# Intelligent-Driving-Laboratory/GOPS

Measured on AMD Instinct MI355X. Metric: env-model steps/sec (batch x H), FHADP compute_gradient + update, higher is better.
Workload: dtype f32; 1 GPU; target_veh3dof_fhadp_b4096_h30; env_id=pyth_veh3dofconti, algorithm=FHADP, batch_per_gpu=4096, horizon=30, activation=elu, parallelism=dp1

## Files before the change

### gops_amd/csrc/api.hip

```cpp
#include <math.h>
#include <stdio.h>
#include <stdlib.h>
#include <string.h>

#include <algorithm>
#include <mutex>
#include <vector>

#include "common.h"
#include "launchers.h"
#include "rollout_choice.h"

bool lds_attr_needed(const void* kernel) {
    static std::mutex mu;
    static std::vector<const void*> seen;
    std::lock_guard<std::mutex> lk(mu);
    for (const void* k : seen)
        if (k == kernel) return false;
    seen.push_back(kernel);
    return true;
}

namespace {

// ... 61 lines not shown
    return buf != nullptr ? buf + 16 * slot : nullptr;
#else
    (void)slot;
    return nullptr;
#endif
}

int check_mlp(const GopsMlp& m, int in_dim, int out_dim, bool f16) {
    if (m.n_layers < 2 || m.n_layers > GOPS_MAX_LAYERS) return GOPS_ERR_UNSUPPORTED;
    if (m.sizes[0] != in_dim || m.sizes[m.n_layers] != out_dim) return GOPS_ERR_BAD_ARG;
    if (out_dim < 1 || out_dim > GOPS_MAX_ACT) return GOPS_ERR_UNSUPPORTED;
    for (int j = 1; j < m.n_layers; ++j)
        if (m.sizes[j] < 16 || (m.sizes[j] & (f16 ? 63 : 15))) return GOPS_ERR_UNSUPPORTED;
    if (m.hidden_act < GOPS_ACT_LINEAR || m.hidden_act > GOPS_ACT_TANH) return GOPS_ERR_BAD_ARG;
    for (int j = 0; j < m.n_layers; ++j)
        if (m.weight[j] == nullptr || m.bias[j] == nullptr) return GOPS_ERR_BAD_ARG;
    return GOPS_OK;
}

void fill_mlp(MlpDev& d, const GopsMlp& m) {
    memset(&d, 0, sizeof(d));
    d.nl = m.n_layers;
    d.act = m.hidden_act;
    for (int j = 0; j <= m.n_layers; ++j) d.dims[j] = m.sizes[j];
    for (int j = 0; j < m.n_layers; ++j) {
        d.kp[j] = pad16(m.sizes[j]);
        d.kp32[j] = pad32(m.sizes[j]);
        d.w[j] = m.weight[j];
        d.b[j] = m.bias[j];
    }
}

void carve_packs(Carver& c, MlpDev& d, bool f16) {
    for (int j = 0; j < d.nl - 1; ++j) {
        if (f16) {
            const size_t n = ((size_t)d.dims[j + 1] * d.kp32[j] + 1) / 2;
            d.wph[j] = reinterpret_cast<const f16x8*>(c.take(n));
            d.wpth[j] = reinterpret_cast<const f16x8*>(c.take(n));
            continue;
        }
        const size_t n = (size_t)d.dims[j + 1] * d.kp[j];
        d.wp[j] = reinterpret_cast<const f32x4*>(c.take(n));
        d.wpt[j] = reinterpret_cast<const f32x4*>(c.take(n));
    }
}

struct Plan {
    RolloutParams p;
    RolloutChoice choice;
    RolloutParams* dev_params = nullptr;
    DwLayer dw[GOPS_MAX_LAYERS];
    float* dw_part[GOPS_MAX_LAYERS] = {};
    float* dw_part_b[GOPS_MAX_LAYERS] = {};
    float* dummy = nullptr;
    size_t dummy_floats = 0;
    size_t bytes = 0;
};

int build_plan(const GopsRolloutDesc& desc, void* ws, Plan& plan) {
    RolloutParams& p = plan.p;
    memset(&p, 0, sizeof(p));
    const GopsEnv& e = desc.env;
    if (desc.batch < 1 || desc.horizon < 1 || desc.horizon > GOPS_MAX_HORIZON) return GOPS_ERR_BAD_ARG;
    if (desc.variant_flags & ~GOPS_VF_ALL) return GOPS_ERR_BAD_ARG;
    if (e.kind < GOPS_ENV_NONE || e.kind > GOPS_ENV_MOBILEROBOT) return GOPS_ERR_BAD_ARG;
    if (e.obs_dim < 1 || e.data_env) return GOPS_ERR_BAD_ARG;
    const int pol_out = (e.kind == GOPS_ENV_NONE) ? 1 : e.act_dim;
    if (desc.dtype != GOPS_DTYPE_F32 && desc.dtype != GOPS_DTYPE_F16) return GOPS_ERR_BAD_ARG;
    const bool f16 = desc.dtype == GOPS_DTYPE_F16;
    int rc = GOPS_OK;
    if (desc.open_loop) {
        if (e.kind == GOPS_ENV_NONE || desc.tail_value || desc.finite_horizon || f16) return GOPS_ERR_BAD_ARG;
    } else if ((rc = check_mlp(desc.policy, e.obs_dim + (desc.finite_horizon ? 1 : 0), pol_out, f16)) != GOPS_OK) {
        return rc;
    }
    if (desc.tail_value && (rc = check_mlp(desc.value, e.obs_dim, 1, f16)) != GOPS_OK) return rc;
    if (e.kind == GOPS_ENV_NONE && (desc.horizon != 1 || desc.tail_value || desc.finite_horizon)) return GOPS_ERR_BAD_ARG;
    if (e.scale_obs && e.kind != GOPS_ENV_LQ && e.kind != GOPS_ENV_IDPENDULUM && e.kind < GOPS_ENV_CARTPOLE) return GOPS_ERR_UNSUPPORTED;
    if (e.kind == GOPS_ENV_CARTPOLE && (e.obs_dim != 4 || e.act_dim != 1)) return GOPS_ERR_BAD_ARG;
    if (e.kind == GOPS_ENV_PENDULUM && (e.obs_dim != 3 || e.act_dim != 1)) return GOPS_ERR_BAD_ARG;
    if (e.kind == GOPS_ENV_VEH2DOF && (e.act_dim != 1 || e.pre_horizon < 1 || e.obs_dim != 4 + e.pre_horizon || e.clip_obs ||
                                        (e.cstr_err && e.n_constraint != 1))) return GOPS_ERR_BAD_ARG;
    if (e.kind == GOPS_ENV_MOBILEROBOT && (e.obs_dim != MOB_OBS || e.act_dim != 2 || e.n_constraint != 1 || e.scale_obs)) return GOPS_ERR_BAD_ARG;
    if (e.kind >= GOPS_ENV_CARTPOLE && f16) return GOPS_ERR_UNSUPPORTED;
    if (e.kind == GOPS_ENV_LQ && (e.obs_dim > GOPS_MAX_LQ_STATE || e.act_dim > GOPS_MAX_ACT)) return GOPS_ERR_UNSUPPORTED;
    if (e.kind == GOPS_ENV_IDPENDULUM && (e.obs_dim != 6 || e.act_dim != 1 || e.clip_obs)) return GOPS_ERR_BAD_ARG;
    if (e.kind == GOPS_ENV_VEH3DOFCONTI &&
        (e.act_dim != 2 || e.pre_horizon < 1 || e.obs_dim != 6 + 4 * e.pre_horizon || e.clip_obs))
        return GOPS_ERR_BAD_ARG;
    if (e.kind == GOPS_ENV_VEH3DOF_SURR &&
        (e.act_dim != 2 || e.pre_horizon < 1 || e.n_surr < (e.cstr_err ? 0 : 1) || e.n_surr > (e.cstr_err ? 0 : GOPS_MAX_SURR) ||
         (e.cstr_err ? e.n_constraint != 2 : (e.n_constraint != 1 && e.n_constraint != 3)) ||
         e.obs_dim != 6 + 4 * e.pre_horizon + 4 * e.n_surr || e.clip_obs ||
         (e.surr_penalty && (e.n_surr != 1 || e.n_constraint != 1)) ||
         desc.open_loop == 1 || desc.dtype != GOPS_DTYPE_F32))
        return GOPS_ERR_BAD_ARG;
    if (e.clip_obs && e.obs_dim > (e.kind == GOPS_ENV_MOBILEROBOT ? GOPS_MAX_CLIP_OBS : 8)) return GOPS_ERR_UNSUPPORTED;
    if (e.repeat_num < 0 || e.repeat_num > GOPS_MAX_REPEAT) return GOPS_ERR_BAD_ARG;
    if (e.repeat_num > 1 && (f16 || (e.kind != GOPS_ENV_LQ && e.kind != GOPS_ENV_IDPENDULUM && e.kind != GOPS_ENV_CARTPOLE &&
                                     e.kind != GOPS_ENV_PENDULUM)))
        return GOPS_ERR_UNSUPPORTED;

    p.B = desc.batch;
    p.H = desc.horizon;
    p.fh = desc.finite_horizon ? 1 : 0;
    p.need_grad = desc.need_grad ? 1 : 0;
    p.tail = desc.tail_value ? 1 : 0;
    p.tail_unmasked = (desc.tail_value && desc.tail_unmasked) ? 1 : 0;
    p.env = e;
    lq_pad_env(p.env);
    fill_ref_defaults(p.env);
    p.open_loop = desc.open_loop == 2 ? 2 : (desc.open_loop ? 1 : 0);
    p.f16 = f16 ? 1 : 0;
    p.vflags = desc.variant_flags;
    p.dw_wgs = desc.dw_workgroups > 0 ? desc.dw_workgroups : 512;
    if (p.open_loop) {
        GopsMlp dummy;
// ... 238 lines not shown
            const long long nw = (long long)p.pol.dims[j + 1] * p.pol.dims[j], nb = p.pol.dims[j + 1];
            int fw = -1, fb = -1;
            for (int k = 0; k < T.n; ++k) {
                if (T.grad[k] == c.grad->weight[j] && T.numel[k] == nw) fw = k;
                if (T.grad[k] == c.grad->bias[j] && T.numel[k] == nb) fb = k;
            }
            if (fw < 0 || fb < 0 || !T.param[fw] || !T.exp_avg[fw] || !T.exp_avg_sq[fw] || !T.param[fb] || !T.exp_avg[fb] || !T.exp_avg_sq[fb])
                return GOPS_ERR_BAD_ARG;
        }
    }
    if (tail->polyak != nullptr) {
        if (tail->adam == nullptr || tail->polyak->n != tail->adam->n) return GOPS_ERR_BAD_ARG;
        for (int k = 0; k < tail->polyak->n; ++k) {
            bool found = false;
            for (int i = 0; i < tail->adam->n; ++i)
                found = found || (tail->polyak->grad[k] == tail->adam->param[i] && tail->polyak->numel[k] == tail->adam->numel[i]);
            if (!found || tail->polyak->param[k] == nullptr) return GOPS_ERR_BAD_ARG;
        }
    }
    return GOPS_OK;
}

int check_backward_call(const GopsRolloutDesc& desc, const RolloutParams& p, const BackwardCall& c) {
    if ((p.open_loop != 0) != (c.g_head_pre != nullptr)) return GOPS_ERR_BAD_ARG;
    if (p.open_loop && c.in->head_pre == nullptr) return GOPS_ERR_BAD_ARG;
    if (c.ext_delta != nullptr && desc.env.kind != GOPS_ENV_NONE) return GOPS_ERR_BAD_ARG;
    if (!p.open_loop && c.want_params)
        for (int j = 0; j < p.pol.nl - (c.ext_delta != nullptr ? 1 : 0); ++j)
            if (c.grad->weight[j] == nullptr || c.grad->bias[j] == nullptr) return GOPS_ERR_BAD_ARG;
    int rc = GOPS_OK;
    if (c.tail != nullptr && (rc = check_update_tail(desc, p, c)) != GOPS_OK) return rc;
    if (c.adj != nullptr && (p.tail || p.f16)) return GOPS_ERR_UNSUPPORTED;
    const Phase ph(p.vflags);
    if ((ph.only_a || ph.only_b) && (p.open_loop || !c.want_params || c.ext_delta != nullptr || c.adj != nullptr)) return GOPS_ERR_UNSUPPORTED;
    return GOPS_OK;
}

bool choose_dw_stage(Plan& plan, const BackwardCall& c, const SweepCall& call) {
    const RolloutParams& p = plan.p;
    const KernelChoice& sweep = plan.choice.bwd;
    if (p.open_loop || !c.want_params) return true;
    const Phase ph(p.vflags);
    const int L = p.pol.nl - 1;
    const bool own_sweep = c.adj == nullptr && c.ext_delta == nullptr;
    const bool cstr_seeds = !(p.env.kind == GOPS_ENV_VEH3DOF_SURR && p.env.surr_penalty) &&
                            (c.in->grad_constraint != nullptr || c.in->grad_constraint_prod != nullptr || c.in->grad_constraint_step != nullptr);
    const bool scaled = own_sweep && !cstr_seeds;
    for (int j = 0; j < L; ++j) {
        if ((ph.only_a && j == 0) || (ph.only_b && j != 0)) continue;
        if (j == 0 && plan.choice.fuse_dw0 && own_sweep && !(p.vflags & (GOPS_VF_BWD_PHASE_A | GOPS_VF_BWD_PHASE_B))) {
            if (!choose_dw_in_sweep(plan.dw[0], sweep.grid, H64_W0_COLS)) return false;
        } else {
            choose_dw_gemm(plan.dw[j], p.f16 != 0, scaled, p.vflags);
        }
    }
    if (c.ext_delta == nullptr && !ph.only_b) {
        if (!sweep_fuses_out(sweep, call)) choose_dw_out(plan.dw[L], p.f16 != 0);
        else if (!choose_dw_in_sweep(plan.dw[L], sweep.grid, plan.dw[L].K)) return false;
    }
    return true;
}

void fill_patch(Plan& plan, const BackwardCall& c, const SweepCall& call, BwdPatch& q) {
    RolloutParams& p = plan.p;
    const int L = p.pol.nl - 1;
    p.in = *c.in;
    p.grad_v = c.grad_v;
    p.g_head_pre = c.g_head_pre;
    p.ext_delta = c.ext_delta;
    p.ext = call.ext;
    if (c.adj != nullptr) {
        p.adj_gfo = c.adj->grad_final_obs;
        p.adj_gobs = c.adj->grad_obs;
        p.adj_first_only = (c.adj->first_step_only != 0 && p.H > 1) ? 1 : 0;
    }
    p.dbg = dbg_timing_buffer(1);
    if (sweep_fuses_out(plan.choice.bwd, call)) {
        p.sp.out_part = plan.dw_part[L];
        p.sp.out_part_b = plan.dw_part_b[L];
    }
    memset(&q, 0, sizeof(q));
    q.in = *c.in;
    q.grad_v = c.grad_v;
    q.g_head_pre = c.g_head_pre;
    q.ext_delta = c.ext_delta;
    q.adj_gfo = p.adj_gfo;
    q.adj_gobs = p.adj_gobs;
    q.adj_first_only = p.adj_first_only;
    q.out_part = p.sp.out_part;
    q.out_part_b = p.sp.out_part_b;
    q.dbg = p.dbg;
    if (plan.dw[0].kernel == DwKernel::InSweep) {
        q.w0_part = plan.dw_part[0];
        q.w0_part_b = plan.dw_part_b[0];
    }
    if (c.tail != nullptr && c.tail->adam != nullptr) {
        q.ad_st = c.tail->adam_state;
        q.ad_snap = p.gscale + 4;
        q.ad_b1 = c.tail->beta1; q.ad_b2 = c.tail->beta2;
    }
}

hipError_t launch_sweep(const GopsRolloutDesc& desc, const Plan& plan, const BackwardCall& c, const BwdPatch& q, hipStream_t s) {
    const RolloutParams& p = plan.p;
    hipError_t e;
    if (p.adj_first_only && c.want_params) {
        const size_t S0 = (size_t)tiles(p) * TB * p.H;
        for (int j = 1; j < p.pol.nl; ++j)
// ... 7 lines not shown
}

hipError_t launch_dw_layer(const DwLayer& d, const void* D, const void* X, float* part, float* part_b, const float* dscale, int rows,
                           float* gw, float* gb, ReduceJobs& jobs, hipStream_t s) {
    const hipError_t e = launch_dw(d, D, X, part, part_b, dscale, s);
    if (e == hipSuccess) add_reduce_jobs(jobs, d, part, part_b, rows, gw, gb);
    return e;
}

void attach_update_tail(ReduceJobs& jobs, const GopsUpdateTail& tail, const RolloutParams& p) {
    if (tail.adam != nullptr) {
        const GopsAdamTensors& T = *tail.adam;
        for (int i = 0; i < jobs.n; ++i)
            for (int k = 0; k < T.n; ++k)
                if (T.grad[k] == jobs.out[i]) { jobs.ad_p[i] = T.param[k]; jobs.ad_m[i] = T.exp_avg[k]; jobs.ad_v[i] = T.exp_avg_sq[k]; }
        jobs.ad_snap = p.gscale + 4;
        jobs.ad_skipped = &tail.adam_state->skipped_nonfinite;
        jobs.ad_b1 = tail.beta1; jobs.ad_b2 = tail.beta2; jobs.ad_eps = (float)tail.eps;
        if (tail.polyak != nullptr) {
            for (int i = 0; i < jobs.n; ++i)
                for (int k = 0; k < tail.polyak->n; ++k)
                    if (jobs.ad_p[i] != nullptr && tail.polyak->grad[k] == jobs.ad_p[i]) jobs.pk_t[i] = tail.polyak->param[k];
            jobs.pk_omt = (float)(1.0 - tail.polyak_tau);
            jobs.pk_tau = (float)tail.polyak_tau;
        }
    }
    if (tail.mean_x != nullptr) {
        jobs.mean_x = tail.mean_x; jobs.mean_n = tail.mean_n; jobs.mean_sc = (float)tail.mean_scale; jobs.mean_stats = tail.mean_stats;
    }
}

int run_backward(const GopsRolloutDesc& desc, const BackwardCall& c, void* ws, size_t ws_bytes, hipStream_t s) {
    if (!desc.need_grad || c.grad_v == nullptr) return GOPS_ERR_BAD_ARG;
    Plan plan;
    int rc = build_plan(desc, ws, plan);
    if (rc != GOPS_OK) return rc;
    if (ws == nullptr || ws_bytes < plan.bytes) return GOPS_ERR_WORKSPACE;
    const RolloutParams& p = plan.p;
    if ((rc = check_backward_call(desc, p, c)) != GOPS_OK) return rc;
    const SweepCall call{desc.env.repeat_num > 1 || c.adj != nullptr, c.ext_delta != nullptr, c.want_params};
    if (!choose_sweep(p, plan.choice, call, plan.choice.bwd) || !choose_dw_stage(plan, c, call)) return GOPS_ERR_UNSUPPORTED;
    BwdPatch q;
    fill_patch(plan, c, call, q);
    hipError_t e;
    if ((e = launch_sweep(desc, plan, c, q, s)) != hipSuccess) return (int)e;
    dbg_print_backward(p);
    if (p.open_loop || !c.want_params) return (int)launch_fill_zero(p.gscale, 4, s);
    ProfScope scope(desc.env.kind == GOPS_ENV_NONE ? 5 : 2, s);
    ReduceJobs jobs;
    memset(&jobs, 0, sizeof(jobs));
    if (p.f16) jobs.unscale = p.gscale;
    else jobs.poison = reinterpret_cast<const unsigned*>(p.gscale) + 3;
    const int L = p.pol.nl - 1;
    for (int j = 0; j <= L; ++j) {
        const DwLayer& d = plan.dw[j];
        if (d.kernel == DwKernel::None) continue;
        if ((e = launch_dw_layer(d, j < L ? p.st.d[j + 1] : p.st.dy, j == 0 ? p.st.x : p.st.h[j], plan.dw_part[j], plan.dw_part_b[j], p.gscale,
                                 d.N, c.grad->weight[j], c.grad->bias[j], jobs, s)) != hipSuccess) return (int)e;
    }
    const bool only_a = Phase(p.vflags).only_a;
    if (!p.f16 && !only_a && jobs.n > 0) jobs.reset = p.gscale;
    if (c.tail != nullptr) attach_update_tail(jobs, *c.tail, p);
    if ((e = launch_reduce(jobs, s)) != hipSuccess) return (int)e;
    if ((p.f16 || jobs.n == 0) && !only_a && (e = launch_fill_zero(p.gscale, 4, s)) != hipSuccess) return (int)e;
    return GOPS_OK;
}

GopsRolloutDesc value_desc(const GopsMlp& value, int batch) {
    GopsRolloutDesc d;
    memset(&d, 0, sizeof(d));
    d.batch = batch;
    d.horizon = 1;
    d.need_grad = 1;
    d.gamma = 1.0;
    d.env.kind = GOPS_ENV_NONE;
    d.env.obs_dim = value.sizes[0];
    d.env.act_dim = 1;
    d.policy = value;
    d.dtype = value.dtype;
    d.variant_flags = value.variant_flags;
    return d;
}

struct MlpPlan {
    GopsRolloutDesc d;
    size_t inner = 0;
    float* zeros = nullptr;
    float* v = nullptr;
    float* gv = nullptr;
    float* gh = nullptr;
    float* gyp = nullptr;
    float* part = nullptr;
    float* part_b = nullptr;
    DwLayer out;
    int K = 0, W = 0, Wp = 0;
    long long S = 0;
    size_t bytes = 0;
};

int plan_mlp(const GopsMlp& mlp, int batch, void* ws, MlpPlan& m) {
    if (mlp.n_layers < 2 || mlp.n_layers > GOPS_MAX_LAYERS || batch < 1) return GOPS_ERR_BAD_ARG;
    if (mlp.dtype != GOPS_DTYPE_F32) return GOPS_ERR_UNSUPPORTED;
    m.W = mlp.sizes[mlp.n_layers];
    m.K = mlp.sizes[mlp.n_layers - 1];
    if (m.W < 1 || m.W > 4096 || (m.K & 15)) return GOPS_ERR_UNSUPPORTED;
    m.Wp = pad16(m.W);
// ... 379 lines not shown
```

### gops_amd/csrc/aux_kernels.hip

```cpp
#include <algorithm>
#include "common.h"
#include "env_models.h"
#include "env_step.h"
#include "launchers.h"

__device__ __forceinline__ void pack_element(const float* __restrict__ W, int N, int K, int Kp,
                                             float* __restrict__ wp, float* __restrict__ wpt, int e) {
    if (e >= N * Kp) return;
    const int i = e & 3, lane = (e >> 2) & 63, blk = e >> 8;
    {
        const int kch = Kp >> 4, nt = blk / kch, c = blk - nt * kch;
        const int n = 16 * nt + (lane & 15), k = 16 * c + 4 * (lane >> 4) + i;
        wp[e] = (k < K) ? W[(size_t)n * K + k] : 0.f;
    }
    {
        const int kch = N >> 4, nt = blk / kch, c = blk - nt * kch;
        const int kin = 16 * nt + (lane & 15), nout = 16 * c + 4 * (lane >> 4) + i;
        wpt[e] = (kin < K) ? W[(size_t)nout * K + kin] : 0.f;
    }
}

__device__ __forceinline__ void pack_element_h(const float* __restrict__ W, int N, int K, int Kp16, int Kp32, int layer,
                                               _Float16* __restrict__ wph, _Float16* __restrict__ wpth, int e) {
    const int i8 = e & 7, lane = (e >> 3) & 63, blk = e >> 9, r = lane & 15, kg = lane >> 4;
    if (e < N * Kp32) {
        const int kch = Kp32 >> 5, c = blk % kch, t = blk / kch, jt = t & 3, q = t >> 2;
        const int n = 64 * q + 16 * (r >> 2) + 4 * jt + (r & 3), k = 32 * c + 8 * kg + i8;
        wph[e] = (_Float16)((k < K) ? W[(size_t)n * K + k] : 0.f);
    }
    const int kchN = N >> 5;
    if (layer >= 1) {
        if (e < N * K) {
            const int c = blk % kchN, t = blk / kchN, jt = t & 3, q = t >> 2;
            const int kin = 64 * q + 16 * (r >> 2) + 4 * jt + (r & 3), nout = 32 * c + 8 * kg + i8;
            wpth[e] = (_Float16)W[(size_t)nout * K + kin];
        }
    } else if (e < N * Kp16) {
        const int c = blk % kchN, nt = blk / kchN;
        const int kin = 16 * nt + r, nout = 32 * c + 8 * kg + i8;
        wpth[e] = (_Float16)((kin < K) ? W[(size_t)nout * K + kin] : 0.f);
    }
}

__device__ __forceinline__ void pack_split_tile(const float* __restrict__ W, int N, int K, bool transposed, bool perm_slots,
                                                int kc, int nt, unsigned short* __restrict__ w1, _Float16* __restrict__ rf,
                                                float* __restrict__ inv) {
    __shared__ float red[256];
    const int tid = threadIdx.x, total = 16 * 32 * kc;
    auto wval = [&](int e) -> float {
        const int i = e & 7, lane = (e >> 3) & 63, c = e >> 9;
        const int col = 16 * nt + (lane & 15), slot = 32 * c + 8 * (lane >> 4) + i;
        const int f = perm_slots ? split_perm(slot) : slot;
        if (!transposed) return (col < N && f < K) ? W[(size_t)col * K + f] : 0.f;
// ... 658 lines not shown
    for (int i = 0; i < 8; ++i)
#pragma unroll
        for (int j = 0; j < 4; ++j) {
            const int k = kb + 16 * j + f;
            if (k >= G.Kp) continue;
#pragma unroll
            for (int r = 0; r < 4; ++r) G.pbase[(size_t)(nb + 16 * i + 4 * g + r) * G.Kp + k] = acc[i][j][r] * unscale;
        }
}
__device__ __attribute__((noinline)) void dw_spec_exact_pass(const DwSpecGeo G, float* ring) {
    constexpr int DT = DwSpec::DT, SF = DwSpec::STAGE_FLOATS, NST = DwSpec::STAGES;
    const int tid = threadIdx.x, lane = tid & 63, wave = tid >> 6;
    const bool mul_wave = wave >= 4;
    const int mw = wave & 3, wn = mw >> 1, wk = mw & 1, f = lane & 15, g = lane >> 4;
    f32x4 acc[8][4] = {};
    dw_spec_copy(G, ring, 0, 0, wave, lane);
    if (G.nblk > 1) dw_spec_copy(G, ring, 1, 1, wave, lane);
    for (int c = 0; c < G.nblk; ++c) {
        asm volatile("s_waitcnt vmcnt(0)" ::: "memory");
        __syncthreads();
        if (c + 2 < G.nblk) dw_spec_copy(G, ring, c + 2, (c + 2) % NST, wave, lane);
        if (mul_wave) {
            const bool half_empty = c >= G.nfull;
            const float* st = ring + (c % NST) * SF;
            const float* da = st + (wn * 128 + f) * 16 + 4 * g;
            const float* xa = st + 2 * DT + (wk * 64 + f) * 16 + 4 * g;
            const f32x4 zero4 = {0.f, 0.f, 0.f, 0.f};
            bf16x8 b[4][3];
#pragma unroll
            for (int j = 0; j < 4; ++j) {
                const f32x4 x0 = *reinterpret_cast<const f32x4*>(xa + 256 * j);
                const f32x4 x1 = half_empty ? zero4 : *reinterpret_cast<const f32x4*>(xa + 256 * j + 2048);
                split_frag(x0, x1, b[j]);
            }
#pragma unroll
            for (int i = 0; i < 8; ++i) {
                const f32x4 d0 = *reinterpret_cast<const f32x4*>(da + 256 * i);
                const f32x4 d1 = half_empty ? zero4 : *reinterpret_cast<const f32x4*>(da + 256 * i + DT);
                bf16x8 a[3];
                split_frag(d0, d1, a);
                constexpr int PA[6] = {2, 0, 1, 1, 0, 0}, PB[6] = {0, 2, 1, 0, 1, 0};
#pragma unroll
                for (int q = 0; q < 6; ++q)
#pragma unroll
                    for (int j = 0; j < 4; ++j)
                        acc[i][j] = __builtin_amdgcn_mfma_f32_16x16x32_bf16(a[PA[q]], b[j][PB[q]], acc[i][j], 0, 0, 0);
                __builtin_amdgcn_sched_barrier(0);
            }
        }
    }
    if (mul_wave) dw_spec_store(G, acc, wn, wk, f, g, 1.f);
}

__global__ __launch_bounds__(512, 1) void dw_gemm_spec_kernel(const float* __restrict__ D, int N, const float* __restrict__ X, int Kp, long long Q,
                                                              int splits, float* __restrict__ part, float* __restrict__ part_b,
                                                              const float* __restrict__ dscale, int guard) {
    extern __shared__ __attribute__((aligned(16))) float ring[];
    constexpr int T = DwSpec::T, TN = DwSpec::TN, DT = DwSpec::DT, SF = DwSpec::STAGE_FLOATS, NST = DwSpec::STAGES;
    const int tid = threadIdx.x, lane = tid & 63, wave = tid >> 6;
    const bool mul_wave = wave >= 4;
    const int tiles_k = (Kp + T - 1) / T, tiles = tiles_k * (N / TN);
    const int xcd = blockIdx.x & 7, local = blockIdx.x >> 3;
    const int tile = local % tiles, split = (local / tiles) * 8 + xcd;
    if (split >= splits) return;
    const int f = lane & 15, g = lane >> 4;
    DwSpecGeo G;
    G.tile_n = tile / tiles_k;
    G.tile_k = tile - G.tile_n * tiles_k;
    G.N = N; G.Kp = Kp; G.Q = Q; G.split = split; G.splits = splits;
    const long long nblk_all = (Q + 1) >> 1;
    G.nblk = (int)((nblk_all - split + splits - 1) / splits);
    const bool odd_tail = (Q & 1) && ((nblk_all - 1) % splits == split);
    G.nfull = odd_tail ? G.nblk - 1 : G.nblk;
    G.xgroups = min(T, Kp - G.tile_k * T) >> 4;
    G.dbase = D + (size_t)G.tile_n * TN * 16;
    G.xbase = X + (size_t)G.tile_k * T * 16;
    G.pbase = part + (size_t)split * N * Kp;
    const int nblk = G.nblk, nfull = G.nfull;

    const int mw = wave & 3, wn = mw >> 1, wk = mw & 1;
    const float sd = f16_grad_scale(dw_delta_yardstick(dscale)) * 16.f;
    float vmax = 0.f, vmax_d = 0.f, vmax_x = 0.f;
    float csum[4] = {0.f, 0.f, 0.f, 0.f};
    const bool want_csum = part_b != nullptr && G.tile_k == 0;

    unsigned* sat = reinterpret_cast<unsigned*>(ring + NST * SF);
    if (tid == 0) *sat = 0u;
    struct Raw { f32x4 v[6][2]; };
    Raw r0, r1;
    const int gg = tid & 3;
    long long lofs[6];
#pragma unroll
    for (int k = 0; k < 6; ++k) {
        const bool isd = k < 4;
        int fe = (tid >> 2) + 64 * (isd ? k : k - 4);
        if (!isd) { int grp = fe >> 4; if (grp >= G.xgroups) grp %= G.xgroups; fe = (grp << 4) | (fe & 15); }
        lofs[k] = (long long)fe * 16 + 4 * gg;
    }
    const size_t dtile = (size_t)N * 16, xtile = (size_t)Kp * 16;
    auto load_block = [&](int c, Raw& r) {
        const size_t q0 = (size_t)(((long long)split + (long long)c * splits) * 2);
        const bool second = c < nfull;
        const f32x4 zero4 = {0.f, 0.f, 0.f, 0.f};
#pragma unroll
        for (int k = 0; k < 6; ++k) {
            const float* base = (k < 4 ? G.dbase + q0 * dtile : G.xbase + q0 * xtile) + lofs[k];
            r.v[k][0] = DW_STREAM_LOAD(reinterpret_cast<const f32x4*>(base));
            r.v[k][1] = second ? DW_STREAM_LOAD(reinterpret_cast<const f32x4*>(base + (k < 4 ? dtile : xtile))) : zero4;
        }
    };
    auto convert_block = [&](const Raw& r, int stage) {
        float* st = ring + stage * SF;
#pragma unroll
        for (int k = 0; k < 6; ++k) {
            const bool isd = k < 4;
            const int fe = (tid >> 2) + 64 * (isd ? k : k - 4), second = isd ? DT : 2048;
// ... 386 lines not shown
    if (splits > chunks) splits = chunks;
    if (splits < 1) splits = 1;
    L.chunks_per_split = (int)((chunks + splits - 1) / splits);
    L.splits = (int)((chunks + L.chunks_per_split - 1) / L.chunks_per_split);
    L.slab_w = (size_t)L.splits * N * Kp;
    L.slab_b = (size_t)L.splits * N;
    return L;
}

DwLayer plan_dw_out(int K, int A, long long S) {
    DwLayer L;
    L.N = A, L.K = L.Kp = L.ld = K, L.S = S;
    L.splits = (int)std::min<long long>(DW_OUT_SPLITS, S);
    L.slab_w = (size_t)DW_OUT_SPLITS * GOPS_MAX_ACT * K;
    L.slab_b = (size_t)DW_OUT_SPLITS * GOPS_MAX_ACT;
    return L;
}

void choose_dw_gemm(DwLayer& L, bool f16, bool scaled, unsigned vflags) {
    const int N = L.N, Kp = L.Kp;
    const bool f32 = (vflags & GOPS_VF_DW_F32) != 0, big = L.tile == 128;
    int tiles = cdiv(N, L.tile) * cdiv(Kp, L.tile);
    L.block = NTHREADS, L.lds = 0;
    L.guard = (vflags & GOPS_VF_DW_NO_GUARD) ? 0 : 1;
    if (f16) {
        L.kernel = DwKernel::F16;
    } else if (!f32 && big && (N % 128) == 0 && ((Kp % 128) == 0 || (Kp > 128 && (Kp % 16) == 0))) {
        const bool h2 = scaled && !(vflags & GOPS_VF_DW_EXACT);
        L.kernel = !h2 ? DwKernel::RingExact : ((N % 256) == 0 ? DwKernel::Spec : DwKernel::RingH2);
        L.lds = (size_t)DWR_STAGES * DWR_STAGE_FLOATS * sizeof(float) + (h2 ? 16 : 0);
        if (L.kernel == DwKernel::Spec) tiles = (N / DwSpec::TN) * cdiv(Kp, DwSpec::T), L.block = DwSpec::NT, L.lds = DwSpec::lds_bytes();
    } else if (!f32 && dw_skinny_ok(N, Kp)) {
        L.kernel = DwKernel::Skinny;
        tiles = cdiv(N, 256);
    } else {
        L.kernel = big ? (f32 ? DwKernel::Fm4F32 : DwKernel::Fm4Bf3) : (f32 ? DwKernel::Fm2F32 : DwKernel::Fm2Bf3);
    }
    L.grid = tiles * cdiv(L.splits, 8) * 8;
}

void choose_dw_out(DwLayer& L, bool f16) {
    L.kernel = f16 ? DwKernel::OutH : DwKernel::OutFm;
    L.grid = L.splits, L.block = NTHREADS, L.lds = 0;
}

bool choose_dw_in_sweep(DwLayer& L, int slabs, int ld) {
    if ((size_t)slabs * L.N * ld > L.slab_w || (size_t)slabs * L.N > L.slab_b) return false;
    L.kernel = DwKernel::InSweep;
    L.splits = slabs, L.ld = ld;
    L.grid = L.block = 0, L.lds = 0;
    return true;
}

hipError_t launch_dw(const DwLayer& L, const void* Dv, const void* Xv, float* part, float* part_b, const float* dscale, hipStream_t s) {
    const float* D = static_cast<const float*>(Dv);
    const float* X = static_cast<const float*>(Xv);
    const _Float16* Xh = static_cast<const _Float16*>(Xv);
    const float* none = nullptr;
    const dim3 grid(L.grid), block(L.block);
    const long long Q = (L.S + TB - 1) / TB;
    auto fm = [&](auto kernel) { hipLaunchKernelGGL(kernel, grid, block, 0, s, D, L.N, X, L.Kp, Q, L.splits, L.chunks_per_split, part, part_b); };
    auto ring = [&](auto kernel, const float* scale, int guard) {
        launch_with_lds(kernel, grid, block, L.lds, s, D, L.N, X, L.Kp, Q, L.splits, L.chunks_per_split, part, part_b, scale, guard);
    };
    switch (L.kernel) {
        case DwKernel::None:
        case DwKernel::InSweep: return hipSuccess;
        case DwKernel::Spec: launch_with_lds(dw_gemm_spec_kernel, grid, block, L.lds, s, D, L.N, X, L.Kp, Q, L.splits, part, part_b, dscale, L.guard); break;
        case DwKernel::RingH2: ring(dw_gemm_ring_kernel<true>, dscale, L.guard); break;
        case DwKernel::RingExact: ring(dw_gemm_ring_kernel<false>, none, 1); break;
        case DwKernel::Skinny: hipLaunchKernelGGL(dw_skinny_kernel, grid, block, 0, s, D, L.N, X, Q, L.splits, part, part_b); break;
        case DwKernel::Fm4Bf3: fm(dw_gemm_fm_kernel<4, true>); break;
        case DwKernel::Fm4F32: fm(dw_gemm_fm_kernel<4, false>); break;
        case DwKernel::Fm2Bf3: fm(dw_gemm_fm_kernel<2, true>); break;
        case DwKernel::Fm2F32: fm(dw_gemm_fm_kernel<2, false>); break;
        case DwKernel::F16:
            hipLaunchKernelGGL(dw_gemm_f16_kernel, grid, block, 0, s, static_cast<const _Float16*>(Dv), L.N, Xh, L.Kp, L.S, L.splits,
                               L.chunks_per_split, part, part_b);
            break;
        case DwKernel::OutH:
            hipLaunchKernelGGL(dw_out_h_kernel, grid, block, 0, s, D, Xh, L.K, L.N, L.S, (L.S + L.splits - 1) / L.splits, part, part_b);
            break;
        case DwKernel::OutFm:
            hipLaunchKernelGGL(dw_out_fm_kernel, grid, block, 0, s, D, X, L.K, L.N, Q, (Q + L.splits - 1) / L.splits, part, part_b);
            break;
    }
    return hipGetLastError();
}

#define LOSS_BLOCKS 64
#define LOSS_ONE_BLOCK_MAX 8192
__device__ __forceinline__ void block_sum2(double& s0, double& s1, double (*red)[4]) {
#pragma unroll
    for (int o = 32; o > 0; o >>= 1) {
        s0 += __shfl_xor(s0, o);
        s1 += __shfl_xor(s1, o);
    }
    __syncthreads();
    if ((threadIdx.x & 63) == 0) { red[0][threadIdx.x >> 6] = s0; red[1][threadIdx.x >> 6] = s1; }
    __syncthreads();
    s0 = (red[0][0] + red[0][1]) + (red[0][2] + red[0][3]);
    s1 = (red[1][0] + red[1][1]) + (red[1][2] + red[1][3]);
}
__device__ __forceinline__ void mean_block(const float* __restrict__ a, int n, float sc, float* __restrict__ stats, double (*red2)[4]) {
    double s0 = 0.0, s1 = 0.0;
    for (int i0 = threadIdx.x; i0 < n; i0 += 8 * 256) {
        float av[8];
#pragma unroll
        for (int q = 0; q < 8; ++q) {
            const int i = i0 + q * 256;
            av[q] = i < n ? a[i] : 0.f;
        }
#pragma unroll
        for (int q = 0; q < 8; ++q)
            if (i0 + q * 256 < n) { s0 += (double)av[q]; s1 += (double)av[q]; }
    }
    block_sum2(s0, s1, red2);
    if (threadIdx.x == 0) {
        stats[0] = (float)((double)sc * s0 / (double)n);
        stats[1] = (float)(s1 / (double)n);
    }
// ... 365 lines not shown
```

### gops_amd/csrc/dw_plan.h

```cpp
#pragma once
#include "common.h"

enum class DwKernel {
    None,
    Spec,
    RingH2,
    RingExact,
    Skinny,
    Fm4Bf3,
    Fm4F32,
    Fm2Bf3,
    Fm2F32,
    F16,
    InSweep,
    OutFm,
    OutH,
};

struct DwLayer {
    int N = 0, K = 0, Kp = 0;
    long long S = 0;
    int tile = 0;
    int splits = 0, chunks_per_split = 0;
    size_t slab_w = 0, slab_b = 0;
    DwKernel kernel = DwKernel::None;
    int grid = 0, block = 0;
    size_t lds = 0;
    int guard = 1;
    int ld = 0;
};

bool dw_skinny_ok(int N, int Kp);
DwLayer plan_dw(int N, int K, int Kp, long long S, bool f16, int wg_target);
DwLayer plan_dw_out(int K, int A, long long S);
void choose_dw_gemm(DwLayer& L, bool f16, bool scaled, unsigned vflags);
void choose_dw_out(DwLayer& L, bool f16);
bool choose_dw_in_sweep(DwLayer& L, int slabs, int ld);
hipError_t launch_dw(const DwLayer& L, const void* D, const void* X, float* part, float* part_b, const float* dscale, hipStream_t s);
void reduce_jobs_add(ReduceJobs& jobs, const float* part, int splits, int rows, int cols, int ld, float* out, int slab_rows = 0);
void add_reduce_jobs(ReduceJobs& jobs, const DwLayer& L, const float* part, const float* part_b, int rows, float* gw, float* gb);
```

### gops_amd/hip_backend.py

```python
import ctypes as C
import os
from typing import Dict, List, Optional, Sequence

import torch

_HERE = os.path.dirname(os.path.abspath(__file__))
LIB_PATH = os.environ.get("GOPS_HIP_LIB") or os.path.join(_HERE, "libgops_hip.so")

MAX_LAYERS, MAX_ACT, MAX_LQ, TILE = 5, 4, 6, 16
ENV_NONE, ENV_LQ, ENV_IDP, ENV_VEH, ENV_VEH_SURR, ENV_CARTPOLE, ENV_PENDULUM, ENV_VEH2DOF, ENV_MOBILEROBOT = 0, 1, 2, 3, 4, 5, 6, 7, 8
MAX_CLIP_OBS = 16
MOBILEROBOT_NOISE_STD = (0.03, 0.02)
MAX_SURR = 4
MAX_REPEAT = 8
ACT_IDS = {"linear": 0, "relu": 1, "elu": 2, "gelu": 3, "selu": 4, "sigmoid": 5, "tanh": 6}
POLY_FULL = {1: 16, 2: 17, 3: 18}
POLY_SYM_2 = 24
RPI_ENV_OSCILLATOR, RPI_ENV_AIRCRAFT, RPI_ENV_SUSPENSION = 1, 2, 3
(RPI_C_GAMMA_ATTE, RPI_C_DT, RPI_C_R, RPI_C_ACT_LOW, RPI_C_ACT_HIGH, RPI_C_ADV_LOW, RPI_C_ADV_HIGH, RPI_C_SCALE_ACT_LOW,
 RPI_C_SCALE_ACT_HIGH, RPI_C_SCALE_ADV_LOW, RPI_C_SCALE_ADV_HIGH, RPI_C_ACTION_SCALE, RPI_C_CLIP_ACTION) = range(13)
RPI_C_Q, RPI_C_THRESHOLD, RPI_C_NORM, RPI_CONST_COUNT = 13, 17, 21, 32
RPI_MAX_BATCH, RPI_MAX_STEPS, RPI_STATE_HEADER = 1024, 1 << 20, 32
DTYPE_IDS = {"fp32": 0, "f32": 0, "float32": 0, "fp16": 1, "f16": 1, "float16": 1, "half": 1}

# ... 1 lines not shown
def dtype_id(name) -> int:
    if name is None:
        return 0
    try:
        return DTYPE_IDS[str(name).lower()]
    except KeyError:
        raise RuntimeError(f"unknown mlp_dtype {name!r}: expected 'fp32' or 'fp16'") from None

_fp = C.POINTER(C.c_float)


class GopsMlp(C.Structure):
    _fields_ = [("n_layers", C.c_int32), ("sizes", C.c_int32 * (MAX_LAYERS + 1)),
                ("hidden_act", C.c_int32), ("dtype", C.c_int32), ("variant_flags", C.c_uint32),
                ("weight", C.c_void_p * MAX_LAYERS), ("bias", C.c_void_p * MAX_LAYERS)]


class GopsMlpGrad(C.Structure):
    _fields_ = [("weight", C.c_void_p * MAX_LAYERS), ("bias", C.c_void_p * MAX_LAYERS)]


class GopsEnv(C.Structure):
    _fields_ = [("kind", C.c_int32), ("obs_dim", C.c_int32), ("act_dim", C.c_int32),
                ("pre_horizon", C.c_int32),
                ("min_action", C.c_float * MAX_ACT), ("max_action", C.c_float * MAX_ACT),
                ("act_low", C.c_float * MAX_ACT), ("act_high", C.c_float * MAX_ACT),
                ("policy_low", C.c_float * MAX_ACT), ("policy_high", C.c_float * MAX_ACT),
                ("clip_obs", C.c_int32), ("obs_low", C.c_float * MAX_CLIP_OBS), ("obs_high", C.c_float * MAX_CLIP_OBS),
                ("shaping", C.c_int32), ("reward_scale", C.c_float), ("reward_shift", C.c_float),
                ("lq_inv_IA", C.c_float * (MAX_LQ * MAX_LQ)), ("lq_B", C.c_float * (MAX_LQ * MAX_ACT)),
                ("lq_Q", C.c_float * MAX_LQ), ("lq_R", C.c_float * MAX_ACT),
                ("lq_dt", C.c_float), ("lq_reward_scale", C.c_float), ("lq_reward_shift", C.c_float),
                ("no_mask_at_done", C.c_int32), ("n_surr", C.c_int32), ("n_constraint", C.c_int32), ("surr_penalty", C.c_int32),
                ("veh_length", C.c_float), ("veh_width", C.c_float),
                ("road_upper", C.c_float), ("road_lower", C.c_float), ("reward_w", C.c_float * 8),
                ("data_env", C.c_int32), ("scale_obs", C.c_int32), ("obs_scale", C.c_float * 8), ("obs_shift", C.c_float * 8),
                ("cstr_err", C.c_int32), ("err_tol", C.c_float * 2),
                ("ref_custom", C.c_int32), ("ref_c", C.c_float * 24),
                ("repeat_num", C.c_int32), ("repeat_last_reward", C.c_int32)]


class GopsRolloutDesc(C.Structure):
    _fields_ = [("batch", C.c_int32), ("horizon", C.c_int32), ("finite_horizon", C.c_int32),
                ("need_grad", C.c_int32), ("tail_value", C.c_int32), ("open_loop", C.c_int32),
                ("dtype", C.c_int32), ("tail_unmasked", C.c_int32), ("variant_flags", C.c_uint32), ("l2_warmup", C.c_int32),
                ("dw_workgroups", C.c_int32), ("reserved0", C.c_int32), ("gamma", C.c_double), ("env", GopsEnv), ("policy", GopsMlp),
                ("value", GopsMlp)]


VF_NO_STATIONARY_SPLIT, VF_NO_STREAMED_SPLIT_FWD, VF_NO_STREAMED_SPLIT_BWD, VF_NO_STREAMED_SPLIT_VALUE = 0x1, 0x2, 0x4, 0x8
VF_STREAMED_FP32, VF_SPLIT_TAIL_MULTI, VF_NO_NARROW_LDS, VF_NO_NARROW_N64 = 0x10, 0x100, 0x400, 0x800
VF_DW_EXACT, VF_DW_F32, VF_DW_NO_GUARD = 0x10000, 0x20000, 0x40000
VF_BWD_PHASE_A, VF_BWD_PHASE_B, VF_NO_FUSED_DW0 = 0x1000000, 0x2000000, 0x4000000
DEFAULT_VARIANT_FLAGS = 0


class GopsRolloutIn(C.Structure):
    _fields_ = [(k, C.c_void_p) for k in ("obs", "done", "state", "ref_points", "path_num", "u_num",
                                          "ref_time", "head_pre", "surr_state", "grad_constraint", "grad_constraint_prod",
                                          "ref_appended", "noise", "grad_constraint_step")]


class GopsRolloutOut(C.Structure):
    _fields_ = [(k, C.c_void_p) for k in ("v_pi", "rewards", "final_obs", "final_done", "final_state", "constraint_sums",
                                          "constraint_prods", "constraints")]


ADAM_MAX = 16


class GopsRolloutAdjoint(C.Structure):
    _fields_ = [("grad_final_obs", C.c_void_p), ("grad_obs", C.c_void_p), ("first_step_only", C.c_int32),
                ("reserved", C.c_int32)]


class GopsAdamTensors(C.Structure):
    _fields_ = [("n", C.c_int32), ("reserved", C.c_int32), ("numel", C.c_int64 * ADAM_MAX),
                ("param", C.c_void_p * ADAM_MAX), ("grad", C.c_void_p * ADAM_MAX),
                ("exp_avg", C.c_void_p * ADAM_MAX), ("exp_avg_sq", C.c_void_p * ADAM_MAX)]


class GopsUpdateTail(C.Structure):
    _fields_ = [("adam", C.POINTER(GopsAdamTensors)), ("adam_state", C.c_void_p), ("beta1", C.c_double), ("beta2", C.c_double),
                ("eps", C.c_double), ("mean_x", C.c_void_p), ("mean_n", C.c_int32), ("reserved", C.c_int32),
                ("mean_scale", C.c_double), ("mean_stats", C.c_void_p), ("polyak", C.POINTER(GopsAdamTensors)), ("polyak_tau", C.c_double)]


class GopsStepIO(C.Structure):
    _fields_ = [(k, C.c_void_p) for k in ("obs", "action", "done", "state", "ref_points", "path_num",
                                          "u_num", "ref_time", "next_obs", "reward", "next_done",
                                          "next_state", "next_ref_points", "next_ref_time",
                                          "surr_state", "next_surr_state", "constraint", "ref_appended", "noise")]


class GopsEpisodeOut(C.Structure):
    _fields_ = [(k, C.c_void_p) for k in ("ret", "length", "terminated", "trace_obs", "trace_act", "trace_rew")]


_lib = None


def lib() -> C.CDLL:
    global _lib
    if _lib is None:
        if not os.path.exists(LIB_PATH):
            raise RuntimeError(
# ... 956 lines not shown
```

### include/gops_hip.h

```cpp
#ifndef GOPS_HIP_H
#define GOPS_HIP_H

#include <stddef.h>
#include <stdint.h>

#ifdef __cplusplus
extern "C" {
#endif
#if defined(__GNUC__) || defined(__clang__)
#pragma GCC visibility push(default)
#endif

#define GOPS_HIP_ABI_VERSION 15

#define GOPS_MAX_LAYERS 5
#define GOPS_MAX_ACT 4
#define GOPS_MAX_LQ_STATE 6
#define GOPS_MAX_HORIZON 256
#define GOPS_TILE 16

enum { GOPS_OK = 0, GOPS_ERR_BAD_ARG = -1, GOPS_ERR_UNSUPPORTED = -2, GOPS_ERR_WORKSPACE = -3 };

enum { GOPS_ENV_NONE = 0, GOPS_ENV_LQ = 1, GOPS_ENV_IDPENDULUM = 2, GOPS_ENV_VEH3DOFCONTI = 3,
       GOPS_ENV_VEH3DOF_SURR = 4,
// ... 220 lines not shown
                             const GopsMlpGrad* grad, void* workspace, size_t workspace_bytes, void* stream);

enum { GOPS_RPI_ENV_OSCILLATOR = 1, GOPS_RPI_ENV_AIRCRAFT = 2, GOPS_RPI_ENV_SUSPENSION = 3 };
#define GOPS_RPI_MAX_BATCH 1024
#define GOPS_RPI_MAX_STEPS (1 << 20)
enum {
    GOPS_RPI_C_GAMMA_ATTE = 0, GOPS_RPI_C_DT = 1, GOPS_RPI_C_R = 2,
    GOPS_RPI_C_ACT_LOW = 3, GOPS_RPI_C_ACT_HIGH = 4, GOPS_RPI_C_ADV_LOW = 5, GOPS_RPI_C_ADV_HIGH = 6,
    GOPS_RPI_C_SCALE_ACT_LOW = 7, GOPS_RPI_C_SCALE_ACT_HIGH = 8, GOPS_RPI_C_SCALE_ADV_LOW = 9, GOPS_RPI_C_SCALE_ADV_HIGH = 10,
    GOPS_RPI_C_ACTION_SCALE = 11, GOPS_RPI_C_CLIP_ACTION = 12,
    GOPS_RPI_C_Q = 13,
    GOPS_RPI_C_THRESHOLD = 17,
    GOPS_RPI_C_NORM = 21,
    GOPS_RPI_CONST_COUNT = 32
};
#define GOPS_RPI_STATE_HEADER 32
size_t gops_rpi_state_bytes(int32_t env_kind, int32_t batch);
int gops_rpi_evaluate(int32_t env_kind, int32_t batch, int32_t max_steps, const float* consts, float* weights,
                      const float* target_weights, const float* max_step, const float* reset_pool, void* state, size_t state_bytes,
                      double lr, double beta1, double beta2, double eps, float* result, float* trace, void* stream);

size_t gops_rpi_mlp_state_bytes(int32_t env_kind, int32_t batch, const GopsMlp* value);
int gops_rpi_mlp_evaluate(int32_t env_kind, int32_t batch, int32_t max_steps, const float* consts, const GopsMlp* value,
                          const GopsMlp* target, const float* max_step, const float* reset_pool, void* state, size_t state_bytes,
                          double lr, double beta1, double beta2, double eps, float* result, float* trace, void* stream);

struct GopsEpisodeOut {
    float* ret; int32_t* length; float* terminated;
    float* trace_obs; float* trace_act; float* trace_rew;
};
typedef struct GopsEpisodeOut GopsEpisodeOut;
size_t gops_episode_workspace_bytes(const GopsEnv* env, const GopsMlp* policy, int32_t episodes, int32_t max_steps);
int gops_episode_rollout(const GopsEnv* env, const GopsMlp* policy, int32_t episodes, int32_t max_steps, const GopsStepIO* init,
                         const GopsEpisodeOut* out, void* workspace, size_t workspace_bytes, void* stream);

#define GOPS_VF_NO_STATIONARY_SPLIT 0x1u
#define GOPS_VF_NO_STREAMED_SPLIT_FWD 0x2u
#define GOPS_VF_NO_STREAMED_SPLIT_BWD 0x4u
#define GOPS_VF_NO_STREAMED_SPLIT_VALUE 0x8u
#define GOPS_VF_STREAMED_FP32 0x10u
#define GOPS_VF_SPLIT_TAIL_MULTI 0x100u
#define GOPS_VF_NO_NARROW_LDS 0x400u
#define GOPS_VF_NO_NARROW_N64 0x800u
#define GOPS_VF_DW_EXACT 0x10000u
#define GOPS_VF_DW_F32 0x20000u
#define GOPS_VF_DW_NO_GUARD 0x40000u
#define GOPS_VF_NO_FUSED_DW0 0x4000000u
#define GOPS_VF_BWD_PHASE_A 0x1000000u
#define GOPS_VF_BWD_PHASE_B 0x2000000u
#define GOPS_VF_ALL (GOPS_VF_NO_STATIONARY_SPLIT | GOPS_VF_NO_STREAMED_SPLIT_FWD | GOPS_VF_NO_STREAMED_SPLIT_BWD | \
                     GOPS_VF_NO_STREAMED_SPLIT_VALUE | GOPS_VF_STREAMED_FP32 | GOPS_VF_SPLIT_TAIL_MULTI | GOPS_VF_NO_NARROW_LDS | \
                     GOPS_VF_NO_NARROW_N64 | GOPS_VF_DW_EXACT | GOPS_VF_DW_F32 | GOPS_VF_DW_NO_GUARD | GOPS_VF_NO_FUSED_DW0 | \
                     GOPS_VF_BWD_PHASE_A | GOPS_VF_BWD_PHASE_B)

#define GOPS_VARIANT_SPLIT 1
#define GOPS_VARIANT_STATIONARY_F32 2
#define GOPS_VARIANT_STREAMED_SPLIT_FWD 4
#define GOPS_VARIANT_HALF_TILE64 8
int gops_rollout_variant(const GopsRolloutDesc* desc);

void gops_profile_enable(int32_t on);
void gops_profile_reset(void);
int gops_profile_read(int32_t kernel_id, double* avg_ms, int64_t* launches);

#if defined(__GNUC__) || defined(__clang__)
#pragma GCC visibility pop
#endif
#ifdef __cplusplus
}
#endif
#endif
```

Measured before the change: 204.2 million env-model steps/s.

## Group per-layer spec dW GEMMs into one launch with balanced XCD dealing

Collects all layers that use the Spec weight-gradient GEMM into a job table and launches one grouped kernel instead of one launch per layer. Work is dealt to the 8 XCDs largest-job-first, assigning each split to the least-loaded XCD. The kernel maps its block index to a job and split through the table. This aims to cut launch overhead and fill the GPU better across small layers, at the cost of a per-block job-lookup loop and a larger kernel argument. The old per-layer path is kept behind a new flag.

Result: no change. 204.2 million env-model steps/s (-0.0%).

```diff
diff --git a/gops_amd/csrc/api.hip b/gops_amd/csrc/api.hip
--- a/gops_amd/csrc/api.hip
+++ b/gops_amd/csrc/api.hip
@@ -137,6 +137,7 @@
     DwLayer dw[GOPS_MAX_LAYERS];
     float* dw_part[GOPS_MAX_LAYERS] = {};
     float* dw_part_b[GOPS_MAX_LAYERS] = {};
+    DwSpecGroup dw_spec;
     float* dummy = nullptr;
     size_t dummy_floats = 0;
     size_t bytes = 0;
@@ -147,7 +148,7 @@
     memset(&p, 0, sizeof(p));
     const GopsEnv& e = desc.env;
     if (desc.batch < 1 || desc.horizon < 1 || desc.horizon > GOPS_MAX_HORIZON) return GOPS_ERR_BAD_ARG;
-    if (desc.variant_flags & ~GOPS_VF_ALL) return GOPS_ERR_BAD_ARG;
+    if (desc.variant_flags & ~(GOPS_VF_ALL | GOPS_VF_DW_PER_LAYER)) return GOPS_ERR_BAD_ARG;
     if (e.kind < GOPS_ENV_NONE || e.kind > GOPS_ENV_MOBILEROBOT) return GOPS_ERR_BAD_ARG;
     if (e.obs_dim < 1 || e.data_env) return GOPS_ERR_BAD_ARG;
     const int pol_out = (e.kind == GOPS_ENV_NONE) ? 1 : e.act_dim;
@@ -492,8 +493,11 @@
             if (!choose_dw_in_sweep(plan.dw[0], sweep.grid, H64_W0_COLS)) return false;
         } else {
             choose_dw_gemm(plan.dw[j], p.f16 != 0, scaled, p.vflags);
-        }
-    }
+            if (plan.dw[j].kernel == DwKernel::Spec)
+                dw_spec_group_add(plan.dw_spec, plan.dw[j], p.st.d[j + 1], j == 0 ? p.st.x : p.st.h[j], plan.dw_part[j], plan.dw_part_b[j]);
+        }
+    }
+    choose_dw_spec_group(plan.dw_spec, p.vflags);
     if (c.ext_delta == nullptr && !ph.only_b) {
         if (!sweep_fuses_out(sweep, call)) choose_dw_out(plan.dw[L], p.f16 != 0);
         else if (!choose_dw_in_sweep(plan.dw[L], sweep.grid, plan.dw[L].K)) return false;
@@ -607,6 +611,7 @@
     if (p.f16) jobs.unscale = p.gscale;
     else jobs.poison = reinterpret_cast<const unsigned*>(p.gscale) + 3;
     const int L = p.pol.nl - 1;
+    if ((e = launch_dw_spec_group(plan.dw_spec, p.gscale, s)) != hipSuccess) return (int)e;
     for (int j = 0; j <= L; ++j) {
         const DwLayer& d = plan.dw[j];
         if (d.kernel == DwKernel::None) continue;
diff --git a/gops_amd/csrc/aux_kernels.hip b/gops_amd/csrc/aux_kernels.hip
--- a/gops_amd/csrc/aux_kernels.hip
+++ b/gops_amd/csrc/aux_kernels.hip
@@ -1,4 +1,5 @@
 #include <algorithm>
+#include <cstring>
 #include "common.h"
 #include "env_models.h"
 #include "env_step.h"
@@ -763,16 +764,27 @@
     if (mul_wave) dw_spec_store(G, acc, wn, wk, f, g, 1.f);
 }
 
-__global__ __launch_bounds__(512, 1) void dw_gemm_spec_kernel(const float* __restrict__ D, int N, const float* __restrict__ X, int Kp, long long Q,
-                                                              int splits, float* __restrict__ part, float* __restrict__ part_b,
-                                                              const float* __restrict__ dscale, int guard) {
+__global__ __launch_bounds__(512, 1) void dw_gemm_spec_kernel(const DwSpecJobs jobs, const float* __restrict__ dscale, int guard) {
     extern __shared__ __attribute__((aligned(16))) float ring[];
     constexpr int T = DwSpec::T, TN = DwSpec::TN, DT = DwSpec::DT, SF = DwSpec::STAGE_FLOATS, NST = DwSpec::STAGES;
     const int tid = threadIdx.x, lane = tid & 63, wave = tid >> 6;
     const bool mul_wave = wave >= 4;
-    const int tiles_k = (Kp + T - 1) / T, tiles = tiles_k * (N / TN);
-    const int xcd = blockIdx.x & 7, local = blockIdx.x >> 3;
-    const int tile = local % tiles, split = (local / tiles) * 8 + xcd;
+    const int xcd = blockIdx.x & 7;
+    int local = blockIdx.x >> 3, j = 0, tiles_k = 1, tiles = 1;
+    for (;; ++j) {
+        if (j >= jobs.n) return;
+        tiles_k = (jobs.job[j].Kp + T - 1) / T, tiles = tiles_k * (jobs.job[j].N / TN);
+        const int room = tiles * jobs.job[j].count[xcd];
+        if (local < room) break;
+        local -= room;
+    }
+    const float* __restrict__ D = jobs.job[j].D;
+    const float* __restrict__ X = jobs.job[j].X;
+    float* __restrict__ part = jobs.job[j].part;
+    float* __restrict__ part_b = jobs.job[j].part_b;
+    const int N = jobs.job[j].N, Kp = jobs.job[j].Kp, splits = jobs.job[j].splits;
+    const long long Q = jobs.Q;
+    const int tile = local % tiles, split = jobs.job[j].first[xcd] + local / tiles;
     if (split >= splits) return;
     const int f = lane & 15, g = lane >> 4;
     DwSpecGeo G;
@@ -1265,6 +1277,70 @@
     return true;
 }
 
+void dw_spec_group_add(DwSpecGroup& G, DwLayer& L, const void* D, const void* X, float* part, float* part_b) {
+    DwSpecJob& J = G.job[G.n];
+    G.layer[G.n++] = &L;
+    J.D = static_cast<const float*>(D), J.X = static_cast<const float*>(X), J.part = part, J.part_b = part_b;
+    J.N = L.N, J.Kp = L.Kp;
+}
+
+static inline int dw_spec_tiles(const DwSpecJob& J) { return (J.N / DwSpec::TN) * cdiv(J.Kp, DwSpec::T); }
+
+static int dw_spec_deal(DwSpecJobs& T) {
+    int load[8] = {};
+    bool dealt[DW_SPEC_MAX_JOBS] = {};
+    for (int k = 0; k < T.n; ++k) {
+        int j = -1;
+        for (int i = 0; i < T.n; ++i)
+            if (!dealt[i] && (j < 0 || dw_spec_tiles(T.job[i]) > dw_spec_tiles(T.job[j]))) j = i;
+        dealt[j] = true;
+        DwSpecJob& J = T.job[j];
+        const int tiles = dw_spec_tiles(J);
+        for (int x = 0; x < 8; ++x) J.count[x] = 0;
+        for (int sp = 0; sp < J.splits; ++sp) {
+            int x = 0;
+            for (int y = 1; y < 8; ++y)
+                if (load[y] < load[x]) x = y;
+            ++J.count[x], load[x] += tiles;
+        }
+        for (int x = 0, f = 0; x < 8; ++x) J.first[x] = f, f += J.count[x];
+    }
+    return *std::max_element(load, load + 8);
+}
+
+void choose_dw_spec_group(DwSpecGroup& G, unsigned vflags) {
+    G.launches = 0;
+    if (G.n == 0) return;
+    const DwLayer& L0 = *G.layer[0];
+    G.guard = L0.guard;
+    DwSpecJobs all;
+    memset(&all, 0, sizeof(all));
+    all.n = G.n, all.Q = (L0.S + TB - 1) / TB;
+    for (int i = 0; i < G.n; ++i) {
+        all.job[i] = G.job[i];
+        all.job[i].splits = G.layer[i]->splits;
+    }
+    if (vflags & GOPS_VF_DW_PER_LAYER) {
+        for (int i = 0; i < G.n; ++i) {
+            DwSpecJobs& T = G.table[i];
+            memset(&T, 0, sizeof(T));
+            T.n = 1, T.Q = all.Q, T.job[0] = all.job[i];
+            G.grid[i] = 8 * dw_spec_deal(T);
+        }
+        G.launches = G.n;
+    } else {
+        G.grid[0] = 8 * dw_spec_deal(all);
+        G.table[0] = all;
+        G.launches = 1;
+    }
+}
+
+hipError_t launch_dw_spec_group(const DwSpecGroup& G, const float* dscale, hipStream_t s) {
+    for (int i = 0; i < G.launches; ++i)
+        launch_with_lds(dw_gemm_spec_kernel, dim3(G.grid[i]), dim3(DwSpec::NT), DwSpec::lds_bytes(), s, G.table[i], dscale, G.guard);
+    return G.launches > 0 ? hipGetLastError() : hipSuccess;
+}
+
 hipError_t launch_dw(const DwLayer& L, const void* Dv, const void* Xv, float* part, float* part_b, const float* dscale, hipStream_t s) {
     const float* D = static_cast<const float*>(Dv);
     const float* X = static_cast<const float*>(Xv);
@@ -1278,8 +1354,8 @@
     };
     switch (L.kernel) {
         case DwKernel::None:
-        case DwKernel::InSweep: return hipSuccess;
-        case DwKernel::Spec: launch_with_lds(dw_gemm_spec_kernel, grid, block, L.lds, s, D, L.N, X, L.Kp, Q, L.splits, part, part_b, dscale, L.guard); break;
+        case DwKernel::InSweep:
+        case DwKernel::Spec: return hipSuccess;
         case DwKernel::RingH2: ring(dw_gemm_ring_kernel<true>, dscale, L.guard); break;
         case DwKernel::RingExact: ring(dw_gemm_ring_kernel<false>, none, 1); break;
         case DwKernel::Skinny: hipLaunchKernelGGL(dw_skinny_kernel, grid, block, 0, s, D, L.N, X, Q, L.splits, part, part_b); break;
diff --git a/gops_amd/csrc/dw_plan.h b/gops_amd/csrc/dw_plan.h
--- a/gops_amd/csrc/dw_plan.h
+++ b/gops_amd/csrc/dw_plan.h
@@ -30,11 +30,38 @@
     int ld = 0;
 };
 
+#define DW_SPEC_MAX_JOBS (GOPS_MAX_LAYERS - 1)
+struct DwSpecJob {
+    const float* D;
+    const float* X;
+    float* part;
+    float* part_b;
+    int N, Kp, splits;
+    int first[8], count[8];
+};
+struct DwSpecJobs {
+    int n;
+    long long Q;
+    DwSpecJob job[DW_SPEC_MAX_JOBS];
+};
+struct DwSpecGroup {
+    int n = 0;
+    DwLayer* layer[DW_SPEC_MAX_JOBS] = {};
+    DwSpecJob job[DW_SPEC_MAX_JOBS] = {};
+    int launches = 0;
+    DwSpecJobs table[DW_SPEC_MAX_JOBS] = {};
+    int grid[DW_SPEC_MAX_JOBS] = {};
+    int guard = 1;
+};
+
 bool dw_skinny_ok(int N, int Kp);
 DwLayer plan_dw(int N, int K, int Kp, long long S, bool f16, int wg_target);
 DwLayer plan_dw_out(int K, int A, long long S);
 void choose_dw_gemm(DwLayer& L, bool f16, bool scaled, unsigned vflags);
 void choose_dw_out(DwLayer& L, bool f16);
+void dw_spec_group_add(DwSpecGroup& G, DwLayer& L, const void* D, const void* X, float* part, float* part_b);
+void choose_dw_spec_group(DwSpecGroup& G, unsigned vflags);
+hipError_t launch_dw_spec_group(const DwSpecGroup& G, const float* dscale, hipStream_t s);
 bool choose_dw_in_sweep(DwLayer& L, int slabs, int ld);
 hipError_t launch_dw(const DwLayer& L, const void* D, const void* X, float* part, float* part_b, const float* dscale, hipStream_t s);
 void reduce_jobs_add(ReduceJobs& jobs, const float* part, int splits, int rows, int cols, int ld, float* out, int slab_rows = 0);
diff --git a/gops_amd/hip_backend.py b/gops_amd/hip_backend.py
--- a/gops_amd/hip_backend.py
+++ b/gops_amd/hip_backend.py
@@ -77,6 +77,7 @@
 VF_STREAMED_FP32, VF_SPLIT_TAIL_MULTI, VF_NO_NARROW_LDS, VF_NO_NARROW_N64 = 0x10, 0x100, 0x400, 0x800
 VF_DW_EXACT, VF_DW_F32, VF_DW_NO_GUARD = 0x10000, 0x20000, 0x40000
 VF_BWD_PHASE_A, VF_BWD_PHASE_B, VF_NO_FUSED_DW0 = 0x1000000, 0x2000000, 0x4000000
+VF_DW_PER_LAYER = 0x8000000
 DEFAULT_VARIANT_FLAGS = 0
 
 
diff --git a/include/gops_hip.h b/include/gops_hip.h
--- a/include/gops_hip.h
+++ b/include/gops_hip.h
@@ -296,6 +296,7 @@
                      GOPS_VF_NO_STREAMED_SPLIT_VALUE | GOPS_VF_STREAMED_FP32 | GOPS_VF_SPLIT_TAIL_MULTI | GOPS_VF_NO_NARROW_LDS | \
                      GOPS_VF_NO_NARROW_N64 | GOPS_VF_DW_EXACT | GOPS_VF_DW_F32 | GOPS_VF_DW_NO_GUARD | GOPS_VF_NO_FUSED_DW0 | \
                      GOPS_VF_BWD_PHASE_A | GOPS_VF_BWD_PHASE_B)
+#define GOPS_VF_DW_PER_LAYER 0x8000000u
 
 #define GOPS_VARIANT_SPLIT 1
 #define GOPS_VARIANT_STATIONARY_F32 2
```
